# MartinPippel/DAmar

Hardware: AMD Instinct MI355X
Metric: aligned base-pairs/sec (daligner block-vs-block) (higher is better)
Workload: dtype int32

## Files before the change

### damar_amd/csrc/kernels/kernels.h

```cpp
#ifndef DAMAR_KERNELS_H
#define DAMAR_KERNELS_H

#include "dev_common.h"

size_t damar_scan_workspace_bytes(u64 n);
void   damar_exclusive_scan_u32(const u32 *in, u32 *out, u64 n, void *work, u64 *total_dev, hipStream_t st);
#define DAMAR_SCAN_TILE 4096
void   damar_tile_offsets_u32(const u32 *in, u64 n, void *work, u64 *total_dev, hipStream_t st);
void   damar_scan_tile_counts(u32 *tcount, u32 ntiles, u64 *total_dev, hipStream_t st);
size_t damar_sort_workspace_bytes(u64 n);
void   damar_sort_set_threads(int threads);
const u32 *damar_sort_error_word(const void *work);
int    damar_radix_sort_keys_u64(u64 *k0, u64 *k1, u64 n, int lobit, int hibit, void *work, hipStream_t st);
void   damar_radix_sort_split_u64(u64 *k0, u64 *k1, u64 n, int lobit, int hibit, u32 *ohi, u32 *olo, void *work,
                                  hipStream_t st);
int    damar_radix_sort_u32(u32 *k0, u32 *v0, u32 *k1, u32 *v1, u64 n, int nbits, void *work, hipStream_t st);
int    damar_radix_sort_keys_u32(u32 *k0, u32 *k1, u64 n, int nbits, void *work, hipStream_t st);
int    damar_radix_sort_u64(u64 *k0, u32 *v0, u64 *k1, u32 *v1, u64 n, int nbits, void *work, hipStream_t st);

enum { DAMAR_PILE_COVER = 0, DAMAR_PILE_REPEAT = 1, DAMAR_PILE_TANDEM = 2 };
#define DAMAR_PILE_ERR_RANGE 1u
typedef struct
{
  const long long *pile_off;
// ... 110 lines not shown

void damar_preload_index(void);  void damar_preload_scan(void);  void damar_preload_sort(void);
void damar_preload_merge(void);  void damar_preload_report(void);
void damar_sort_set_prio(int on);
void damar_merge_set_prio(int on);
void damar_index_set_prio(int on);
void damar_launch_kmer_tuples(const DevBlock *blk, int kmer, u32 nkmers, void *codes, int wide, u32 *pos, hipStream_t st);
void damar_launch_mask_flags(const DevBlock *blk, int kmer, const u32 *pos, u32 n, u32 *keep, hipStream_t st);
void damar_launch_biased_tuples(const DevBlock *blk, int kmer, const int *logbase, void *codes, int wide, u32 *pos,
                                u32 *keep, hipStream_t st);
void damar_launch_suppress_flags(const void *codes, int wide, u32 n, int suppress, u32 *keep, hipStream_t st);
void damar_launch_compact_pairs(const void *k, int wide, const u32 *v, const u32 *keep, const u32 *off, u32 n,
                                void *ko, u32 *vo, hipStream_t st);

void damar_launch_tandem_links(const DevBlock *blk, int kmer, const void *codes, int wide, const u32 *pos, u32 n,
                               int *dist, hipStream_t st);

typedef struct
{ const void *acode;  const u32 *apos;  u32 alen;
  const void *bcode;  const u32 *bpos;  u32 blen;
  int  wide;
  int  kbits;
  int  self, comp, identity;
  u32  limit;
  DevBlock ablk, bblk;
  int  pbits, abits;
  int  dbits;
  u32  b_lo, b_hi;
} MergeArgs;

typedef struct { u32 b0, b1, ja, ia;
                 u32 sh, pad[3]; } MergeTile;

size_t damar_merge_workspace_bytes(u32 alen);
u32   *damar_merge_tile_counts(void *work, u32 alen);
u32    damar_merge_tiles(u32 alen);
void   damar_launch_merge_count(const MergeArgs *m, void *work, unsigned long long *gram, u32 ngram, hipStream_t st);
void damar_launch_merge_emit(const MergeArgs *m, void *work, u64 nhits, u64 *keys, u32 *vals, u32 *pid, hipStream_t st);
void damar_launch_merge_bread_hist(const MergeArgs *m, void *work, unsigned long long *hist, hipStream_t st);
void damar_launch_merge_range(const MergeArgs *m, void *work, hipStream_t st);
void damar_launch_pair_heads_ids(const u32 *pids, u64 nhits, u64 off, u64 gtotal, int abits, int minhit, int nshift,
                                 u64 *send, u64 *bits, void *scan_work, u64 *total_dev, u32 *heads, hipStream_t st);
void damar_launch_pair_bitmap(const u32 *pids, const u32 *heads, u32 nheads, int abits, u32 b_lo, u32 b_hi, u32 *bitmap,
                              hipStream_t st);
void damar_launch_seed_cut_count(const u64 *keys, u64 nhits, int pbits, const u32 *bitmap, u32 *tcount, u64 *total_dev,
                                 hipStream_t st);
void damar_launch_seed_cut_scatter(const u64 *keys, const u32 *vals, u64 nhits, int pbits, const u32 *bitmap,
                                   const u32 *toff, u64 *okeys, u32 *ovals, hipStream_t st);
void damar_launch_pair_heads(const u64 *keys, u64 nhits, u64 off, u64 gtotal, int pbits, int abits, int minhit, int nshift,
                             u64 *send , u64 *bits, void *scan_work, u64 *total_dev,
                             u32 *heads, hipStream_t st);
void damar_launch_pair_work(u64 *keys, const u32 *vals, u64 nhits, u64 off, u64 gtotal, int ppos, int dbits, int abits, int minhit, int nshift,
                            u64 *send , u64 *bits, void *scan_work, u64 *total_dev ,
                            int binshift, int kmer, int hitmin, u32 b_lo, u32 b_hi, int unsorted, hipStream_t st);
size_t damar_order_runs_scratch_bytes(u64 nhits);
void damar_launch_order_runs(u64 *keys, u64 nhits, int ppos, int dbits, const u32 *work, u32 nwork, void *scratch, hipStream_t st);
void damar_launch_pair_work_expand(const u64 *bits, const void *scan_work, u64 nhits, u32 *work, hipStream_t st);
#define WORK_COST_BITS 16
#define WORK_COST_MAX  ((1u << WORK_COST_BITS) - 1)
void damar_launch_work_cost(const u64 *keys, const u32 *vals, u64 nhits, int pbits, int abits, int dbits, const u32 *aboff,
                            const u32 *bboff, const u32 *work, u32 nwork, u32 coarse, u32 *key, u32 *val, hipStream_t st);
void damar_launch_pair_screen(const u64 *keys, const u32 *vals, u64 nhits, int pbits, int dbits, const u32 *heads, u32 nheads,
                              int minhit, int binshift, int kmer, int hitmin, int abits, u32 b_lo, u32 b_hi, u32 *keep, hipStream_t st);
void damar_launch_compact_u32(const u32 *src, const u32 *keep, const u32 *off, u32 n, u32 *out, hipStream_t st);
void damar_launch_compact_index(const u32 *flags, const u32 *off, u64 n, u32 *out, hipStream_t st);

#ifdef __HIPCC__
__device__ __forceinline__ int seed_diag(u64 k, const u32 *__restrict__ vals, u64 i, u64 pmask, int dbits)
{ if (dbits)
    return (int) ((k >> dbits) & pmask) - (int) (k & ((1ull << dbits) - 1));
  return (int) vals[i];
}
#endif

typedef struct
{ int abpos, bbpos, aepos, bepos, diffs;
  int atlen, btlen;
  int aread, bread;
  u32 item, seq;
  u32 toff;
} LaRecord;

typedef struct
{
  const u64 *keys;  const u32 *vals;  u64 nhits;
  const u32 *work;  u32 nwork;
  DevBlock ablk, bblk;
  int  pbits, abits, dbits;
  int  kmer, hitmin, binshift, minhit;
// ... 134 lines not shown
```

### damar_amd/csrc/kernels/seed_merge.hip

```cpp
#include "dev_common.h"
#include "kernels.h"

SEED_PRIO_VAR(g_merge_prio, 0)
SEED_PRIO_SETTER(damar_merge_set_prio, g_merge_prio)


__device__ __forceinline__ u32 count_below(const u32 *__restrict__ bpos, u32 jb, u32 ib, u32 bound)
{ u32 a = jb, b = ib;
  while (a < b)
    { u32 m = (a + b) >> 1;
      if (bpos[m] < bound) a = m + 1; else b = m;
    }
  return a - jb;
}


#ifndef MT_PER
#define MT_PER  4
#endif
#define MT_A    (MT_PER * 256)
#define MT_BCAP (3 * MT_A)
#define MT_HITS 4
#define MT_NBK  2048

template <typename CodeT>
__device__ __forceinline__ u32 lower_bound_c(const CodeT *c, u32 lo, u32 hi, CodeT x)
{ while (lo < hi)
    { const u32 mid = (lo + hi) >> 1;
      if (c[mid] < x) lo = mid + 1; else hi = mid;
    }
  return lo;
}
template <typename CodeT>
__device__ __forceinline__ u32 upper_bound_c(const CodeT *c, u32 lo, u32 hi, CodeT x)
{ while (lo < hi)
    { const u32 mid = (lo + hi) >> 1;
      if (c[mid] <= x) lo = mid + 1; else hi = mid;
    }
  return lo;
}

#define MT_SMP 8192
template <typename CodeT>
__global__ __launch_bounds__(256)
void merge_tiles(MergeArgs m, u32 ntiles, MergeTile *__restrict__ tiles)
{ SEED_PRIO(g_merge_prio);
  constexpr u32 NS = sizeof(CodeT) == 4 ? MT_SMP : MT_SMP / 2;
  __shared__ CodeT smp[NS];
  const CodeT *acode = (const CodeT *) m.acode, *bcode = (const CodeT *) m.bcode;
  const u32 stride = (m.blen + NS - 1) / NS;
  if (m.blen > 0)
    for (u32 j = threadIdx.x; j < NS; j += 256)
      { const u64 e = (u64) (j + 1) * stride - 1;
        smp[j] = bcode[e < m.blen ? (u32) e : m.blen - 1];
      }
  __syncthreads();
  const u32 t = blockIdx.x * 256u + threadIdx.x;
  if (t >= ntiles)
    return;
  const u32 a0 = t * (u32) MT_A, a1 = min(m.alen, a0 + (u32) MT_A);
  const CodeT c0 = acode[a0], c1 = acode[a1 - 1];
  MergeTile tl;
  tl.b0 = tl.b1 = m.blen;
  if (m.blen > 0)
    { u32 lo = 0, hi = NS;
      while (lo < hi)
        { const u32 mid = (lo + hi) >> 1;
          if (smp[mid] < c0) lo = mid + 1; else hi = mid;
        }
      u32 l0 = m.blen, h0 = m.blen, l1 = m.blen, h1 = m.blen;
      if (lo < NS)
        { const u64 s0 = (u64) lo * stride;
          l0 = (u32) s0;  h0 = (u32) min((u64) m.blen, s0 + stride);
        }
      lo = 0;  hi = NS;
      while (lo < hi)
        { const u32 mid = (lo + hi) >> 1;
          if (smp[mid] <= c1) lo = mid + 1; else hi = mid;
        }
      if (lo < NS)
        { const u64 s0 = (u64) lo * stride;
          l1 = (u32) s0;  h1 = (u32) min((u64) m.blen, s0 + stride);
        }
// ... 318 lines not shown
    }
  if (threadIdx.x == 0)
    tcount[tile] = (T64 > 0xffffffffull) ? 0xffffffffu : (u32) T64;
  typedef u32 V4 __attribute__((ext_vector_type(4)));
  if (nv == MT_PER && MT_PER == 4)
    { V4 vc, vj;
#pragma unroll
      for (int k = 0; k < 4; k++)
        { vc[k] = n[k];  vj[k] = tl.b0 + jb[k]; }
      *(V4 *) (cnt + a0 + e0) = vc;
      *(V4 *) (jbg + a0 + e0) = vj;
    }
  else
    {
#pragma unroll
      for (int k = 0; k < MT_PER; k++)
        if (k < nv)
          { cnt[a0 + e0 + k] = n[k];
            jbg[a0 + e0 + k] = tl.b0 + jb[k];
          }
    }
}

static_assert(MT_BCAP + 16 < (1 << 16), "a packed entry holds the piece-relative start and the hits in 16 bits each");
struct MergeFastArgs
{ const void *acode, *bcode;
  const u32  *apos, *bpos;
  u32 alen, blen;
  int self, identity, comp, rpbits;
};

template <typename CodeT>
__global__ __launch_bounds__(256, 8)
void merge_fast(MergeFastArgs m, MergeTile *__restrict__ tiles, u32 *__restrict__ tcount, u32 *__restrict__ cnt)
{ SEED_PRIO(g_merge_prio);
  __shared__ __attribute__((aligned(16))) CodeT sb[MT_BCAP + 16 / sizeof(CodeT)];
  __shared__ __attribute__((aligned(16))) u16 first[MT_NBK];
  __shared__ u32 wsum[4];
  __shared__ u32 deep;
  const CodeT *acode = (const CodeT *) m.acode, *bcode = (const CodeT *) m.bcode;
  const u32 tile = blockIdx.x;
  const MergeTile tl = tiles[tile];
  const u32 a0 = tile * (u32) MT_A, a1 = min(m.alen, a0 + (u32) MT_A), nat = a1 - a0;
  const u32 nbt = tl.b1 - tl.b0;
  if (nbt > MT_BCAP || (m.self && m.rpbits == 0))
    { if (threadIdx.x == 0)
        tiles[tile].pad[0] = 1;
      return;
    }
  const u32 e0 = threadIdx.x * MT_PER;
  const int nv = (e0 >= nat) ? 0 : (int) min((u32) MT_PER, nat - e0);
  const u32 sh = tl.sh, nmax = tl.pad[1];
  constexpr u32 VPK = 16 / sizeof(CodeT);
  typedef CodeT VecT __attribute__((ext_vector_type(16 / sizeof(CodeT))));
  typedef u32 V4 __attribute__((ext_vector_type(4)));

  const CodeT c0 = acode[a0];
  CodeT a[MT_PER];
  if (nv == MT_PER)
    {
#pragma unroll
      for (int q = 0; q < MT_PER / (int) VPK; q++)
        { const VecT v = ((const VecT *) (acode + a0 + e0))[q];
#pragma unroll
          for (int e = 0; e < (int) VPK; e++)
            a[q * VPK + e] = v[e];
        }
    }
  else
    {
#pragma unroll
      for (int k = 0; k < MT_PER; k++)
        a[k] = (k < nv) ? acode[a0 + e0 + k] : (CodeT) 0;
    }
  const u32 b0a = tl.b0 & ~(VPK - 1), shf = tl.b0 - b0a;
  { const u32 nvec = (tl.b1 - b0a + VPK - 1) / VPK;
    const u32 whole = (m.blen - b0a) / VPK;
    VecT v[MT_BCAP / (int) VPK / 256 + 1];
#pragma unroll
    for (int r = 0; r < MT_BCAP / (int) VPK / 256 + 1; r++)
// ... 52 lines not shown
                  while (q < nbt && B[q] == c)
                    { q += 1;
                      if (++steps == 4) { q = upper_bound_c<CodeT>(B, q, nbt, c);  break; }
                    }
                  jb[k] = p;  n[k] = q - p;
                }
            }
          longest = max(longest, n[k]);
        }
    }
  if (longest > nmax)
    deep = 1;
  u32 sum = 0;
  if (m.self)
    { const int rp = m.rpbits;
#pragma unroll
      for (int k = 0; k < MT_PER; k++)
        if (n[k] > 0)
          { const u32 p = m.apos[a0 + e0 + k], ra = p >> rp;
            u32 bound = m.identity ? (m.comp ? (ra + 1) << rp : p) : ra << rp;
            if (!(m.identity && m.comp && ((ra + 1) >> (32 - rp)) != 0))
              n[k] = count_below(m.bpos, tl.b0 + jb[k], tl.b0 + jb[k] + n[k], bound);
          }
    }
#pragma unroll
  for (int k = 0; k < MT_PER; k++)
    sum += n[k];
  sum = (u32) wave_sum_i((int) sum);
  if (lane_id() == 0)
    wsum[threadIdx.x >> 6] = sum;
  __syncthreads();
  if (deep)
    { if (threadIdx.x == 0)
        tiles[tile].pad[0] = 1;
      return;
    }
  if (threadIdx.x == 0)
    { tcount[tile] = wsum[0] + wsum[1] + wsum[2] + wsum[3];
      tiles[tile].pad[2] = 1;
    }
  if (nv == MT_PER && MT_PER == 4)
    { V4 vc;
#pragma unroll
      for (int k = 0; k < 4; k++)
        vc[k] = (n[k] << 16) | jb[k];
      *(V4 *) (cnt + a0 + e0) = vc;
    }
  else
    {
#pragma unroll
      for (int k = 0; k < MT_PER; k++)
        if (k < nv)
          cnt[a0 + e0 + k] = (n[k] << 16) | jb[k];
    }
}

template <typename CodeT>
__global__ __launch_bounds__(256, 8)
void merge_sweep(MergeArgs m, const MergeTile *__restrict__ tiles, u32 *__restrict__ tcount, u32 *__restrict__ cnt,
                 u32 *__restrict__ jbg, unsigned long long *__restrict__ gram, u32 ngram, int only_flagged)
{ SEED_PRIO(g_merge_prio);
  __shared__ __attribute__((aligned(16))) CodeT sb[MT_BCAP + 16 / sizeof(CodeT)];
  __shared__ u32 loc[MT_A + 1];
  __shared__ u32 sjb[2];
  __shared__ u32 sw4[4];
  __shared__ u64 red[4];
  const MergeTile tl = tiles[blockIdx.x];
  if (only_flagged && tl.pad[0] == 0)
    return;
  if (tl.b1 - tl.b0 <= MT_BCAP)
    merge_sweep_tile<CodeT, true>(m, tl, blockIdx.x, tcount, cnt, jbg, gram, ngram, sb, loc, sjb, sw4, red);
  else
    merge_sweep_tile<CodeT, false>(m, tl, blockIdx.x, tcount, cnt, jbg, gram, ngram, sb, loc, sjb, sw4, red);
}

__global__ __launch_bounds__(256, 8)
void merge_emit(MergeArgs m, const MergeTile *__restrict__ tiles, const u32 *__restrict__ cnt, const u32 *__restrict__ jbg,
                const u32 *__restrict__ toff, u64 nhits, u64 *__restrict__ keys, u32 *__restrict__ vals, u32 *__restrict__ pid)
{ SEED_PRIO(g_merge_prio);
  __shared__ u32 loc[MT_A + 1];
  __shared__ u32 sjb[MT_A];
  __shared__ u32 sw4[4];
  const int l = lane_id(), w = threadIdx.x >> 6;
  const u32 tile = blockIdx.x;
  const u32 a0 = tile * (u32) MT_A, a1 = min(m.alen, a0 + (u32) MT_A), nat = a1 - a0;
  const u32 e0 = threadIdx.x * MT_PER;
  const u64 h0 = toff[tile];
  const u64 hn = (tile + 1 < gridDim.x) ? (u64) toff[tile + 1] : nhits;
  if (hn == h0)
    return;
  u32 n[MT_PER], s = 0;
  const bool packed = tiles[tile].pad[2] != 0;
  const u32 pb0 = tiles[tile].b0;
#pragma unroll
  for (int k = 0; k < MT_PER; k++)
    { const bool ok = e0 + k < nat;
      const u32 w = ok ? cnt[a0 + e0 + k] : 0;
      n[k] = packed ? w >> 16 : w;
      sjb[e0 + k] = !ok ? 0 : packed ? pb0 + (w & 0xffffu) : jbg[a0 + e0 + k];
      s += n[k];
    }
  u32 inc = (u32) wave_incl_scan_i((int) s);
  if (l == 63) sw4[w] = inc;
  __syncthreads();
  u32 ex = inc - s;
  for (int i = 0; i < 4; i++)
// ... 147 lines not shown
{ SEED_PRIO(g_merge_prio);
  __shared__ u64 red[4];
  const u32 tile = blockIdx.x;
  const u32 a0 = tile * (u32) MT_A, a1 = min(m.alen, a0 + (u32) MT_A);
  const bool packed = tiles[tile].pad[2] != 0;
  const u32 pb0 = tiles[tile].b0;
  u64 sum = 0;
  for (u32 i = a0 + threadIdx.x; i < a1; i += 256)
    { const u32 v = cnt[i];
      const u32 n = packed ? v >> 16 : v;
      if (n == 0)
        continue;
      const u32 jb = packed ? pb0 + (v & 0xffffu) : jbg[i];
      const u32 lo = count_reads_below(m, jb, n, m.b_lo), hi = count_reads_below(m, jb, n, m.b_hi);
      const u32 nn = hi > lo ? hi - lo : 0;
      if (packed)
        cnt[i] = (nn << 16) | (jb + lo - pb0);
      else
        { cnt[i] = nn;
          jbg[i] = jb + lo;
        }
      sum += nn;
    }
  const u64 T64 = block_sum_u64(sum, red);
  if (threadIdx.x == 0)
    tcount[tile] = (T64 > 0xffffffffull) ? 0xffffffffu : (u32) T64;
}


static size_t mw_tiles(u32 alen)  { return ((size_t) alen + MT_A - 1) / MT_A; }
static size_t mw_off_counts(u32 alen) { return (mw_tiles(alen) * sizeof(MergeTile) + 255) & ~(size_t) 255; }
static size_t mw_off_cnt(u32 alen)    { return mw_off_counts(alen) + (((mw_tiles(alen) + 1) * sizeof(u32) + 255) & ~(size_t) 255); }
static size_t mw_off_jb(u32 alen)     { return mw_off_cnt(alen) + (((size_t) alen * sizeof(u32) + 255) & ~(size_t) 255); }

size_t damar_merge_workspace_bytes(u32 alen)
{ return mw_off_jb(alen) + (((size_t) alen * sizeof(u32) + 255) & ~(size_t) 255); }

u32 *damar_merge_tile_counts(void *work, u32 alen) { return (u32 *) ((char *) work + mw_off_counts(alen)); }

u32 damar_merge_tiles(u32 alen) { return (u32) mw_tiles(alen); }

void damar_launch_merge_count(const MergeArgs *m, void *work, unsigned long long *gram, u32 ngram, hipStream_t st)
{ if (m->alen == 0)
    return;
  const u32 ntiles = (u32) mw_tiles(m->alen);
  MergeTile *tiles = (MergeTile *) work;
  u32 *tcount = damar_merge_tile_counts(work, m->alen);
  u32 *cnt = (u32 *) ((char *) work + mw_off_cnt(m->alen)), *jb = (u32 *) ((char *) work + mw_off_jb(m->alen));
  static int general = -1;
  if (general < 0)
    general = getenv("DAMAR_MERGE_GENERAL") != NULL;
  const bool fast = gram == NULL && !general;
  MergeFastArgs f;
  f.acode = m->acode;  f.bcode = m->bcode;  f.apos = m->apos;  f.bpos = m->bpos;  f.alen = m->alen;  f.blen = m->blen;
  f.self = m->self;  f.identity = m->identity;  f.comp = m->comp;  f.rpbits = m->ablk.rpbits;
  if (m->wide)
    { hipLaunchKernelGGL(merge_tiles<u64>, dim3((ntiles + 255) / 256), dim3(256), 0, st, *m, ntiles, tiles);
      if (fast)
        hipLaunchKernelGGL(merge_fast<u64>, dim3(ntiles), dim3(256), 0, st, f, tiles, tcount, cnt);
      hipLaunchKernelGGL(merge_sweep<u64>, dim3(ntiles), dim3(256), 0, st, *m, tiles, tcount, cnt, jb, gram, ngram, fast ? 1 : 0);
    }
  else
    { hipLaunchKernelGGL(merge_tiles<u32>, dim3((ntiles + 255) / 256), dim3(256), 0, st, *m, ntiles, tiles);
      if (fast)
        hipLaunchKernelGGL(merge_fast<u32>, dim3(ntiles), dim3(256), 0, st, f, tiles, tcount, cnt);
      hipLaunchKernelGGL(merge_sweep<u32>, dim3(ntiles), dim3(256), 0, st, *m, tiles, tcount, cnt, jb, gram, ngram, fast ? 1 : 0);
    }
}

void damar_launch_merge_emit(const MergeArgs *m, void *work, u64 nhits, u64 *keys, u32 *vals, u32 *pid, hipStream_t st)
{ if (nhits == 0)
    return;
  const u32 ntiles = (u32) mw_tiles(m->alen);
  const u32 *toff = damar_merge_tile_counts(work, m->alen);
  const u32 *cnt = (const u32 *) ((char *) work + mw_off_cnt(m->alen)), *jb = (const u32 *) ((char *) work + mw_off_jb(m->alen));
  hipLaunchKernelGGL(merge_emit, dim3(ntiles), dim3(256), 0, st, *m, (const MergeTile *) work, cnt, jb, toff, nhits, keys, vals, pid);
}

void damar_launch_merge_bread_hist(const MergeArgs *m, void *work, unsigned long long *hist, hipStream_t st)
{ if (m->alen == 0)
    return;
  const u32 ntiles = (u32) mw_tiles(m->alen);
  const u32 *cnt = (const u32 *) ((char *) work + mw_off_cnt(m->alen)), *jb = (const u32 *) ((char *) work + mw_off_jb(m->alen));
  hipLaunchKernelGGL(merge_bread_hist, dim3(ntiles), dim3(256), 0, st, *m, (const MergeTile *) work, cnt, jb, hist);
}

void damar_launch_merge_range(const MergeArgs *m, void *work, hipStream_t st)
{ if (m->alen == 0)
    return;
  const u32 ntiles = (u32) mw_tiles(m->alen);
  u32 *tcount = damar_merge_tile_counts(work, m->alen);
  u32 *cnt = (u32 *) ((char *) work + mw_off_cnt(m->alen)), *jb = (u32 *) ((char *) work + mw_off_jb(m->alen));
  hipLaunchKernelGGL(merge_range, dim3(ntiles), dim3(256), 0, st, *m, (const MergeTile *) work, tcount, cnt, jb);
}

#define SCREEN_MAX   48
#define SCREEN_PANEL 50000
template <typename K>
__global__ __launch_bounds__(64)
// ... 572 lines not shown
{ u32 n = 0;
  for (;;)
    { const u64 x = i + (u64) n + (u64) l;
      const u64 same = __ballot(x < nhits && (keys[x] >> pshift) == pr);
      if (same != ~0ull)
        return n + (u32) __ffsll((long long) ~same) - 1u;
      n += 64;
      if (n > maxrun)
        return n;
    }
}

__global__ __launch_bounds__(256)
void order_probe(const u64 *__restrict__ keys, u64 nhits, int ppos, int dbits, const u64 *__restrict__ bits, u64 *__restrict__ flag,
                 u32 maxrun)
{ SEED_PRIO(g_merge_prio);
  __shared__ u16 hl[DAMAR_SCAN_TILE];
  __shared__ u32 nh;
  const int  l = lane_id();
  const u64  base = (u64) blockIdx.x * DAMAR_SCAN_TILE;
  if (threadIdx.x == 0)
    nh = 0;
  __syncthreads();
  if (threadIdx.x < DAMAR_SCAN_TILE / 64)
    { u64 w = bits[(base >> 6) + threadIdx.x];
      while (w)
        { const int b = __ffsll((long long) w) - 1;
          w &= w - 1;
          hl[atomicAdd(&nh, 1u)] = (u16) (threadIdx.x * 64u + (u32) b);
        }
    }
  __syncthreads();
  const u32 n_h = nh;
  bool over = false;
  for (u32 h = threadIdx.x >> 6; h < n_h; h += 4)
    { const u64 i = base + hl[h];
      over |= run_length(keys, nhits, i, ppos + dbits, maxrun, l, keys[i] >> (ppos + dbits)) > maxrun;
    }
  if (over && l == 0)
    atomicOr((unsigned long long *) flag, 1ull);
}

template <u32 J>
__device__ __forceinline__ u32 lane_xor(u32 v)
{ if constexpr (J == 1)
    return (u32) __builtin_amdgcn_update_dpp(0, (int) v, 0xB1, 0xf, 0xf, true);
  else if constexpr (J == 2)
    return (u32) __builtin_amdgcn_update_dpp(0, (int) v, 0x4E, 0xf, 0xf, true);
  else if constexpr (J == 8)
    return (u32) __builtin_amdgcn_update_dpp(0, (int) v, 0x128, 0xf, 0xf, true);
  else if constexpr (J == 4 || J == 16)
    return (u32) __builtin_amdgcn_ds_swizzle((int) v, (int) (0x1f | (J << 10)));
  else
    return (u32) __shfl_xor((int) v, (int) J);
}

template <int K, u32 K2, u32 JJ>
__device__ __forceinline__ void or_step(u32 (&c)[K], int l)
{ if constexpr (JJ >= 64)
    {
#pragma unroll
      for (int q = 0; q < K; q++)
        if ((q & (int) (JJ >> 6)) == 0)
          { const int  p  = q | (int) (JJ >> 6);
            const bool up = (((u32) q << 6) & K2) == 0;
            const u32  lo = min(c[q], c[p]), hi = max(c[q], c[p]);
            c[q] = up ? lo : hi;
            c[p] = up ? hi : lo;
          }
    }
  else
    {
#pragma unroll
// ... 126 lines not shown
          { for (u32 t = threadIdx.x; t < (P >> 1); t += 256)
              { const u32 ix = ((t & ~(jj - 1)) << 1) | (t & (jj - 1)), px = ix | jj;
                const bool up = (ix & k2) == 0;
                const u32 a = ck[ix], c = ck[px];
                if ((a > c) == up)
                  { ck[ix] = c;  ck[px] = a; }
              }
            __syncthreads();
          }
      for (u32 j = threadIdx.x; j < n; j += 256)
        keys[i + j] = rk[ck[j] & 2047u];
      __syncthreads();
    }
}

size_t damar_order_runs_scratch_bytes(u64 nhits)
{ return sizeof(u32) * (size_t) (2 * (nhits / (OR_WAVE + 1)) + 2); }

#ifdef OR_STATS
static void or_stats_print(void)
{ unsigned long long h[16];
  if (hipMemcpyFromSymbol(h, HIP_SYMBOL(g_or_hist), sizeof(h)) != hipSuccess)
    return;
  unsigned long long runs = 0;
  for (int b = 0; b <= 12; b++)
    runs += h[b];
  fprintf(stderr, "order_runs: %llu kept runs, %llu seeds in them\n", runs, h[13]);
  for (int b = 0; b <= 12; b++)
    if (h[b])
      fprintf(stderr, "  runs of %5d..%-5d %9llu  (%.3f %%)\n", b == 0 ? 1 : (1 << b) + 1, b == 12 ? 1 << 30 : 2 << b, h[b], 100. * h[b] / runs);
}
#endif

void damar_launch_order_runs(u64 *keys, u64 nhits, int ppos, int dbits, const u32 *work, u32 nwork, void *scratch, hipStream_t st)
{ if (nwork == 0)
    return;
#ifdef OR_STATS
  static int reg = 0;
  if (!reg)
    { reg = 1;  atexit(or_stats_print); }
#endif
  u32 *lcount = (u32 *) scratch;
  HIP_CHECK(hipMemsetAsync(lcount, 0, sizeof(u32), st));
  const u32 slice = std::min<u32>(OR_SLICE, 4u * std::max<u32>(1u, nwork / 2048u));
  hipLaunchKernelGGL(order_waves, dim3((nwork + slice - 1) / slice), dim3(256), 0, st, keys, nhits, ppos, dbits, work, nwork, slice,
                     lcount, lcount + 2);
  if (nhits > OR_WAVE)
    { const u64 most = nhits / (OR_WAVE + 1);
      hipLaunchKernelGGL(order_long, dim3((u32) std::min<u64>(std::min<u64>(nwork, most), 1024)), dim3(256), 0, st, keys, ppos, dbits,
                         (const u32 *) lcount, (const u32 *) (lcount + 2));
    }
}

void damar_launch_pair_work(u64 *keys, const u32 *vals, u64 nhits, u64 off, u64 gtotal, int ppos, int dbits, int abits, int minhit, int nshift,
                            u64 *send, u64 *bits, void *scan_work, u64 *total_dev, int binshift, int kmer, int hitmin,
                            u32 b_lo, u32 b_hi, int unsorted, hipStream_t st)
{ HIP_CHECK(hipMemsetAsync(total_dev, 0, 2 * sizeof(u64), st));
  if (nhits == 0)
    return;
  if (nshift > 6)
    nshift = 6;
  const u32 ntiles = (u32) ((nhits + DAMAR_SCAN_TILE - 1) / DAMAR_SCAN_TILE);
  u32 *tcount = (u32 *) scan_work;
  if (nshift >= 0)
    hipLaunchKernelGGL(slice_ends<u64>, dim3(1), dim3(64), 0, st, keys, nhits, off, gtotal, abits + ppos + dbits, nshift, send);
  if (!unsorted)
    hipLaunchKernelGGL(pair_work_mark<false>, dim3(ntiles), dim3(256), 0, st, (const u64 *) keys, vals, nhits, ppos, dbits, abits, minhit,
                       nshift, (const u64 *) send, binshift, kmer, hitmin, b_lo, b_hi, bits, tcount);
  else
    { hipLaunchKernelGGL(pair_work_mark<true>, dim3(ntiles), dim3(256), 0, st, (const u64 *) keys, vals, nhits, ppos, dbits, abits, minhit,
                         nshift, (const u64 *) send, binshift, kmer, hitmin, b_lo, b_hi, bits, tcount);
      static int maxrun = -1;
      if (maxrun < 0)
        { const char *e = getenv("DAMAR_TEST_RUN_MAX");
          maxrun = (e && atoi(e) >= 2 && atoi(e) <= OR_MAX) ? atoi(e) : OR_MAX;
        }
      hipLaunchKernelGGL(order_probe, dim3(ntiles), dim3(256), 0, st, (const u64 *) keys, nhits, ppos, dbits, (const u64 *) bits, total_dev + 1,
                         (u32) maxrun);
    }
  damar_scan_tile_counts(tcount, ntiles, total_dev, st);
// ... 89 lines not shown
```

### damar_amd/csrc/kernels/sort_scan.hip

```cpp
#include "dev_common.h"
#include "kernels.h"

#define SCAN_THREADS 256
#define SCAN_ITEMS   16
#define SCAN_TILE    (SCAN_THREADS * SCAN_ITEMS)


__device__ __forceinline__ u32 block_excl_scan_256(u32 v, u32 *lds4, u32 *total)
{ int l = lane_id(), w = threadIdx.x >> 6;
  u32 inc = (u32) wave_incl_scan_i((int) v);
  if (l == 63) lds4[w] = inc;
  __syncthreads();
  u32 base = 0, tot = 0;
  for (int i = 0; i < 4; i++)
    { u32 s = lds4[i];
      if (i < w) base += s;
      tot += s;
    }
  __syncthreads();
  *total = tot;
  return base + inc - v;
}

__global__ __launch_bounds__(SCAN_THREADS)
void scan_tile_sums(const u32 *__restrict__ in, u64 n, u32 *__restrict__ tsum)
{ __shared__ u32 lds4[4];
  u64 base = (u64) blockIdx.x * SCAN_TILE + (u64) threadIdx.x * SCAN_ITEMS;
  u32 s = 0;
  for (int i = 0; i < SCAN_ITEMS; i++)
    if (base + i < n) s += in[base + i];
  u32 tot;
  block_excl_scan_256(s, lds4, &tot);
  if (threadIdx.x == 0) tsum[blockIdx.x] = tot;
}

__global__ __launch_bounds__(SCAN_THREADS)
void scan_tile_offsets(u32 *__restrict__ tsum, u32 ntiles, u64 *__restrict__ total)
{ __shared__ u32 lds4[4];
  u64 carry = 0;
  for (u32 b = 0; b < ntiles; b += SCAN_THREADS)
    { u32 i = b + threadIdx.x;
      u32 v = (i < ntiles) ? tsum[i] : 0, tot;
      u32 ex = block_excl_scan_256(v, lds4, &tot);
      if (i < ntiles) tsum[i] = (u32) (carry + ex);
      carry += tot;
    }
  if (threadIdx.x == 0) *total = carry;
}

__global__ __launch_bounds__(SCAN_THREADS)
void scan_tile_apply(const u32 *__restrict__ in, u32 *__restrict__ out, u64 n, const u32 *__restrict__ toff)
{ __shared__ u32 lds4[4];
  u64 base = (u64) blockIdx.x * SCAN_TILE + (u64) threadIdx.x * SCAN_ITEMS;
  u32 v[SCAN_ITEMS], s = 0;
  for (int i = 0; i < SCAN_ITEMS; i++)
    { v[i] = (base + i < n) ? in[base + i] : 0;
      s += v[i];
    }
  u32 tot;
  u32 ex = block_excl_scan_256(s, lds4, &tot) + toff[blockIdx.x];
  for (int i = 0; i < SCAN_ITEMS; i++)
    { if (base + i < n) out[base + i] = ex;
      ex += v[i];
    }
}

size_t damar_scan_workspace_bytes(u64 n)
{ u64 ntiles = (n + SCAN_TILE - 1) / SCAN_TILE;
  return ((((size_t) (ntiles + 1) * sizeof(u32)) + 63) & ~(size_t) 63) + 64;
}

void damar_exclusive_scan_u32(const u32 *in, u32 *out, u64 n, void *work, u64 *total_dev, hipStream_t st)
{ u32 ntiles = (u32) ((n + SCAN_TILE - 1) / SCAN_TILE);
  u32 *tsum = (u32 *) work;
  if (n == 0)
    { HIP_CHECK(hipMemsetAsync(total_dev, 0, sizeof(u64), st));
      return;
// ... 26 lines not shown
```

### damar_amd/csrc/shim.hip

```cpp
#include <algorithm>
#include <vector>
#include <deque>
#include <string>
#include <thread>
#include <atomic>
#include <mutex>
#include <condition_variable>
#include <functional>
#include <string.h>
#include <unistd.h>

#include "kernels/dev_common.h"
#include <ctype.h>
#include "kernels/kernels.h"

extern "C" {
#include "damar_filter.h"
#include "damar_hip.h"
#include "host/damar_host.h"
}

#define MAXGRAM 10000

static void die(void)
// ... 2120 lines not shown
      flags = (u32 *) arena_take(&G_tmp2, sizeof(u32) * (size_t) nsurv);
      foff  = (u32 *) arena_take(&G_tmp2, std::max(sizeof(u32) * (size_t) nsurv, bit_words_bytes(nsurv)));
      scw2  = arena_take(&G_tmp2, damar_scan_workspace_bytes(nsurv));
      sends = (u64 *) arena_take(&G_tmp2, 64 * sizeof(u64));
      damar_launch_seed_cut_scatter(uk, m.dbits ? NULL : uv, total, m.pbits + m.dbits, bitmap, (const u32 *) scc, k0, v0, G_st);
      int side = m.dbits ? damar_radix_sort_keys_u64(k0, k1, nsurv, m.dbits, m.dbits + sbits, sw2, G_st)
                         : damar_radix_sort_u64(k0, v0, k1, v1, nsurv, sbits, sw2, G_st);
      sort_check(sw2);
      keys = side ? k1 : k0;
      vals = side ? v1 : v0;
      if (keys != pk)
        { fprintf(stderr, "damar: internal error, the seed sort ended on the wrong side\n");
          die();
        }
      total  = nsurv;
      hshift = -1;
    }
  stage("seed_sort");
  tick(2);

  u64 nwork64 = 0;
  u32 *work = NULL;
  if (!two_step)
    {
      u64 got[2] = { 0, 0 };
      if (cut)
        psort = false;
      damar_launch_pair_work(keys, vals, total, s_off, s_all, m.pbits, m.dbits, m.abits, minhit, hshift, sends, (u64 *) foff ,
                             scw2, tot, P_binshift, P_kmer, P_hitmin, P_bread_lo, P_bread_hi, psort ? 1 : 0, G_st);
      stage("run_heads");
      tick(3);
      HIP_CHECK(hipMemcpyAsync(got, tot, 2 * sizeof(u64), hipMemcpyDeviceToHost, G_st));
      stream_wait(G_st);
      if (psort && got[1] != 0)
        {
          G_cnt[7] += 1;
          u64 *other = (keys == tk) ? NULL : tk;
          if (other == NULL || resort_ws == NULL)
            { fprintf(stderr, "damar: internal error, no room to sort the seeds again\n");
              die();
            }
          int side = damar_radix_sort_keys_u64(keys, other, total, m.dbits, m.dbits + sbits, resort_ws, G_st);
          sort_check(resort_ws);
          if (side)
            HIP_CHECK(hipMemcpyAsync(keys, other, sizeof(u64) * (size_t) total, hipMemcpyDeviceToDevice, G_st));
          damar_launch_pair_work(keys, vals, total, s_off, s_all, m.pbits, m.dbits, m.abits, minhit, hshift, sends, (u64 *) foff, scw2, tot,
                                 P_binshift, P_kmer, P_hitmin, P_bread_lo, P_bread_hi, 0, G_st);
          HIP_CHECK(hipMemcpyAsync(got, tot, 2 * sizeof(u64), hipMemcpyDeviceToHost, G_st));
          stream_wait(G_st);
          psort = false;
        }
      nwork64 = got[0];
      arena_reserve(&G_ord, 5 * pad256(sizeof(u32) * (size_t) nwork64) + pad256(damar_sort_workspace_bytes(nwork64)) + 8192);
      work = (u32 *) arena_take(&G_ord, sizeof(u32) * ((size_t) nwork64 + 1));
      if (nwork64 > 0)
        { damar_launch_pair_work_expand((const u64 *) foff, scw2, total, work, G_st);
          if (psort)
            damar_launch_order_runs(keys, total, m.pbits, m.dbits, work, (u32) nwork64, order_ws, G_st);
        }
      stage("work_list");
    }
  else
    { u32 *heads = (u32 *) tk;
      damar_launch_pair_heads(keys, total, s_off, s_all, m.pbits + m.dbits, m.abits, minhit, hshift, sends, (u64 *) foff ,
                              scw2, tot, heads, G_st);
      stage("run_heads");
      HIP_CHECK(hipMemcpyAsync(&nwork64, tot, sizeof(u64), hipMemcpyDeviceToHost, G_st));
      HIP_CHECK(hipStreamSynchronize(G_st));
      const u32 nheads = (u32) nwork64;
      arena_reserve(&G_ord, 5 * pad256(sizeof(u32) * (size_t) nheads) + pad256(damar_sort_workspace_bytes(nheads)) + 8192);
      work = (u32 *) arena_take(&G_ord, sizeof(u32) * ((size_t) nheads + 1));
      nwork64 = 0;
      if (nheads > 0)
        { damar_launch_pair_screen(keys, vals, total, m.pbits, m.dbits, heads, nheads, minhit, P_binshift, P_kmer, P_hitmin, m.abits,
                                   P_bread_lo, P_bread_hi, flags, G_st);
          damar_exclusive_scan_u32(flags, foff, nheads, scw2, tot, G_st);
          damar_launch_compact_u32(heads, flags, foff, nheads, work, G_st);
          stage("work_list");
          HIP_CHECK(hipMemcpyAsync(&nwork64, tot, sizeof(u64), hipMemcpyDeviceToHost, G_st));
        }
    }
  if (two_step)
    { tick(3);
      HIP_CHECK(hipStreamSynchronize(G_st));
    }
  sort_verify();
  const u32 nwork = (u32) nwork64;
  G_ms[DAMAR_T_MERGE] += lap(0, 1);
  G_ms[DAMAR_T_SSORT] += lap(1, 2);
  G_ms[DAMAR_T_WORK]  += lap(2, 3);
  G_cnt[0] += nhits;  G_cnt[1] += nwork;
// ... 823 lines not shown
  damar_dev_block *b = damar_block_upload(ablock);
  damar_match_self(ablock, b, settings, NULL);
  damar_block_free(b);
}


extern "C" int damar_last_slabs(int *b_lo, int64 *hits, int cap)
{ const int n = G_plan.n;
  for (int i = 0; i < n && i < cap; i++)
    { if (b_lo) b_lo[i] = G_plan.b_lo[(size_t) i];
      if (hits) hits[i] = G_plan.hits[(size_t) i];
    }
  if (b_lo != NULL && n <= cap && (size_t) n < G_plan.b_lo.size())
    b_lo[n] = G_plan.b_lo[(size_t) n];
  return n;
}

extern "C" void damar_slab_totals(int64 *out)
{ out[0] = G_slab_tot[0];  out[1] = G_slab_tot[1]; }

extern "C" int damar_order_runs_test(uint64 *keys, int64 nhits, int ppos, int dbits, const uint32 *work, int nwork)
{ finish_all();
  ensure_init();
  if (nhits <= 0 || nwork <= 0)
    return 0;
  u64  *dk;
  u32  *dw;
  void *sc;
  HIP_CHECK(hipMalloc((void **) &dk, sizeof(u64) * (size_t) nhits));
  HIP_CHECK(hipMalloc((void **) &dw, sizeof(u32) * (size_t) nwork));
  HIP_CHECK(hipMalloc(&sc, damar_order_runs_scratch_bytes((u64) nhits)));
  HIP_CHECK(hipMemcpy(dk, keys, sizeof(u64) * (size_t) nhits, hipMemcpyHostToDevice));
  HIP_CHECK(hipMemcpy(dw, work, sizeof(u32) * (size_t) nwork, hipMemcpyHostToDevice));
  damar_launch_order_runs(dk, (u64) nhits, ppos, dbits, dw, (u32) nwork, sc, G_st);
  HIP_CHECK(hipStreamSynchronize(G_st));
  HIP_CHECK(hipMemcpy(keys, dk, sizeof(u64) * (size_t) nhits, hipMemcpyDeviceToHost));
  HIP_CHECK(hipFree(dk));  HIP_CHECK(hipFree(dw));  HIP_CHECK(hipFree(sc));
  return 0;
}

extern "C" int64 damar_last_seeds(void *out, int64 cap)
{ struct SP { int diag, apos, aread, bread; } *sp = (SP *) out;
  if (out == NULL)
    { G_keep_seeds = (cap != 0);
      return 0;
    }
  int64 n = (int64) G_seed_keys.size();
  for (int64 i = 0; i < n && i < cap; i++)
    { u64 k = G_seed_keys[(size_t) i];
      const int bpos = (int) (k & ((1ull << G_seed_dbits) - 1));
      k >>= G_seed_dbits;
      sp[i].apos  = (int) (k & ((1ull << G_seed_pbits) - 1));
      sp[i].aread = (int) ((k >> G_seed_pbits) & ((1ull << G_seed_abits) - 1));
      sp[i].bread = (int) (k >> (G_seed_pbits + G_seed_abits));
      sp[i].diag  = G_seed_dbits ? sp[i].apos - bpos : (int) G_seed_vals[(size_t) i];
    }
  return n;
}

extern "C" int damar_local_alignment_batch_opts(damar_dev_block *ablk, damar_dev_block *bblk, int comp,
                                                Align_Spec *spec, const int *tasks, int ntasks,
                                                int *paths, int64 *trace_off, uint16 *traces, int64 trace_cap,
                                                int t8, int *t8_fell_back, int *wide_tasks)
{ finish_all();
  ensure_init();
  if (t8_fell_back) *t8_fell_back = 0;
  if (wide_tasks)   *wide_tasks = 0;
// ... 935 lines not shown
```

Baseline: 53.87 billion.

## Sweep only fallback merge tiles via worklist and skip idle long-run ordering

merge_fast now appends each tile it cannot handle to a device worklist. A grid-strided merge_sweep_list kernel then processes only those tiles, replacing the full-grid merge_sweep launch in which most blocks exit early. The run-length check now sets a separate 'long run' flag bit, so order_long is launched only when some run is longer than a wave. The tile-offset scan is also rewritten to handle several items per thread with u64 accumulation. Both skips can be turned off with an environment variable, and correctness depends on the atomic list and flag bits being set reliably.

```diff
diff --git a/damar_amd/csrc/kernels/kernels.h b/damar_amd/csrc/kernels/kernels.h
--- a/damar_amd/csrc/kernels/kernels.h
+++ b/damar_amd/csrc/kernels/kernels.h
@@ -166,6 +166,7 @@
 typedef struct { u32 b0, b1, ja, ia;
                  u32 sh, pad[3]; } MergeTile;
 
+int    damar_seed_idle_skip(void);
 size_t damar_merge_workspace_bytes(u32 alen);
 u32   *damar_merge_tile_counts(void *work, u32 alen);
 u32    damar_merge_tiles(u32 alen);
@@ -184,11 +185,14 @@
 void damar_launch_pair_heads(const u64 *keys, u64 nhits, u64 off, u64 gtotal, int pbits, int abits, int minhit, int nshift,
                              u64 *send , u64 *bits, void *scan_work, u64 *total_dev,
                              u32 *heads, hipStream_t st);
+#define DAMAR_RUN_OVER 1u
+#define DAMAR_RUN_LONG 2u
 void damar_launch_pair_work(u64 *keys, const u32 *vals, u64 nhits, u64 off, u64 gtotal, int ppos, int dbits, int abits, int minhit, int nshift,
                             u64 *send , u64 *bits, void *scan_work, u64 *total_dev ,
                             int binshift, int kmer, int hitmin, u32 b_lo, u32 b_hi, int unsorted, hipStream_t st);
 size_t damar_order_runs_scratch_bytes(u64 nhits);
-void damar_launch_order_runs(u64 *keys, u64 nhits, int ppos, int dbits, const u32 *work, u32 nwork, void *scratch, hipStream_t st);
+void damar_launch_order_runs(u64 *keys, u64 nhits, int ppos, int dbits, const u32 *work, u32 nwork, void *scratch, int maybe_long,
+                             hipStream_t st);
 void damar_launch_pair_work_expand(const u64 *bits, const void *scan_work, u64 nhits, u32 *work, hipStream_t st);
 #define WORK_COST_BITS 16
 #define WORK_COST_MAX  ((1u << WORK_COST_BITS) - 1)
diff --git a/damar_amd/csrc/kernels/seed_merge.hip b/damar_amd/csrc/kernels/seed_merge.hip
--- a/damar_amd/csrc/kernels/seed_merge.hip
+++ b/damar_amd/csrc/kernels/seed_merge.hip
@@ -3,6 +3,15 @@
 
 SEED_PRIO_VAR(g_merge_prio, 0)
 SEED_PRIO_SETTER(damar_merge_set_prio, g_merge_prio)
+
+int damar_seed_idle_skip(void)
+{ static int on = -1;
+  if (on < 0)
+    { const char *e = getenv("DAMAR_SEED_SKIP");
+      on = (e == NULL || atoi(e) != 0) ? 1 : 0;
+    }
+  return on;
+}
 
 
 __device__ __forceinline__ u32 count_below(const u32 *__restrict__ bpos, u32 jb, u32 ib, u32 bound)
@@ -43,12 +52,14 @@
 #define MT_SMP 8192
 template <typename CodeT>
 __global__ __launch_bounds__(256)
-void merge_tiles(MergeArgs m, u32 ntiles, MergeTile *__restrict__ tiles)
+void merge_tiles(MergeArgs m, u32 ntiles, MergeTile *__restrict__ tiles, u32 *__restrict__ fcount)
 { SEED_PRIO(g_merge_prio);
   constexpr u32 NS = sizeof(CodeT) == 4 ? MT_SMP : MT_SMP / 2;
   __shared__ CodeT smp[NS];
   const CodeT *acode = (const CodeT *) m.acode, *bcode = (const CodeT *) m.bcode;
   const u32 stride = (m.blen + NS - 1) / NS;
+  if (blockIdx.x == 0 && threadIdx.x == 0)
+    *fcount = 0;
   if (m.blen > 0)
     for (u32 j = threadIdx.x; j < NS; j += 256)
       { const u64 e = (u64) (j + 1) * stride - 1;
@@ -433,7 +444,8 @@
 
 template <typename CodeT>
 __global__ __launch_bounds__(256, 8)
-void merge_fast(MergeFastArgs m, MergeTile *__restrict__ tiles, u32 *__restrict__ tcount, u32 *__restrict__ cnt)
+void merge_fast(MergeFastArgs m, MergeTile *__restrict__ tiles, u32 *__restrict__ tcount, u32 *__restrict__ cnt,
+                u32 *__restrict__ fcount, u32 *__restrict__ flist)
 { SEED_PRIO(g_merge_prio);
   __shared__ __attribute__((aligned(16))) CodeT sb[MT_BCAP + 16 / sizeof(CodeT)];
   __shared__ __attribute__((aligned(16))) u16 first[MT_NBK];
@@ -446,7 +458,9 @@
   const u32 nbt = tl.b1 - tl.b0;
   if (nbt > MT_BCAP || (m.self && m.rpbits == 0))
     { if (threadIdx.x == 0)
-        tiles[tile].pad[0] = 1;
+        { tiles[tile].pad[0] = 1;
+          flist[atomicAdd(fcount, 1u)] = tile;
+        }
       return;
     }
   const u32 e0 = threadIdx.x * MT_PER;
@@ -565,7 +579,9 @@
   __syncthreads();
   if (deep)
     { if (threadIdx.x == 0)
-        tiles[tile].pad[0] = 1;
+        { tiles[tile].pad[0] = 1;
+          flist[atomicAdd(fcount, 1u)] = tile;
+        }
       return;
     }
   if (threadIdx.x == 0)
@@ -605,6 +621,29 @@
     merge_sweep_tile<CodeT, true>(m, tl, blockIdx.x, tcount, cnt, jbg, gram, ngram, sb, loc, sjb, sw4, red);
   else
     merge_sweep_tile<CodeT, false>(m, tl, blockIdx.x, tcount, cnt, jbg, gram, ngram, sb, loc, sjb, sw4, red);
+}
+
+#define MT_LIST_GRID 512
+template <typename CodeT>
+__global__ __launch_bounds__(256)
+void merge_sweep_list(MergeArgs m, const MergeTile *__restrict__ tiles, u32 *__restrict__ tcount, u32 *__restrict__ cnt,
+                      u32 *__restrict__ jbg, const u32 *__restrict__ fcount, const u32 *__restrict__ flist)
+{ SEED_PRIO(g_merge_prio);
+  __shared__ __attribute__((aligned(16))) CodeT sb[MT_BCAP + 16 / sizeof(CodeT)];
+  __shared__ u32 loc[MT_A + 1];
+  __shared__ u32 sjb[2];
+  __shared__ u32 sw4[4];
+  __shared__ u64 red[4];
+  const u32 nf = *fcount;
+  for (u32 f = blockIdx.x; f < nf; f += gridDim.x)
+    { const u32 tile = flist[f];
+      const MergeTile tl = tiles[tile];
+      if (tl.b1 - tl.b0 <= MT_BCAP)
+        merge_sweep_tile<CodeT, true>(m, tl, tile, tcount, cnt, jbg, NULL, 0, sb, loc, sjb, sw4, red);
+      else
+        merge_sweep_tile<CodeT, false>(m, tl, tile, tcount, cnt, jbg, NULL, 0, sb, loc, sjb, sw4, red);
+      __syncthreads();
+    }
 }
 
 __global__ __launch_bounds__(256, 8)
@@ -818,9 +857,10 @@
 static size_t mw_off_counts(u32 alen) { return (mw_tiles(alen) * sizeof(MergeTile) + 255) & ~(size_t) 255; }
 static size_t mw_off_cnt(u32 alen)    { return mw_off_counts(alen) + (((mw_tiles(alen) + 1) * sizeof(u32) + 255) & ~(size_t) 255); }
 static size_t mw_off_jb(u32 alen)     { return mw_off_cnt(alen) + (((size_t) alen * sizeof(u32) + 255) & ~(size_t) 255); }
+static size_t mw_off_flag(u32 alen)   { return mw_off_jb(alen) + (((size_t) alen * sizeof(u32) + 255) & ~(size_t) 255); }
 
 size_t damar_merge_workspace_bytes(u32 alen)
-{ return mw_off_jb(alen) + (((size_t) alen * sizeof(u32) + 255) & ~(size_t) 255); }
+{ return mw_off_flag(alen) + (((mw_tiles(alen) + 1) * sizeof(u32) + 255) & ~(size_t) 255); }
 
 u32 *damar_merge_tile_counts(void *work, u32 alen) { return (u32 *) ((char *) work + mw_off_counts(alen)); }
 
@@ -837,20 +877,31 @@
   if (general < 0)
     general = getenv("DAMAR_MERGE_GENERAL") != NULL;
   const bool fast = gram == NULL && !general;
+  const bool listed = fast && damar_seed_idle_skip();
+  u32 *fcount = (u32 *) ((char *) work + mw_off_flag(m->alen)), *flist = fcount + 1;
+  const u32 lgrid = std::min<u32>(ntiles, MT_LIST_GRID);
   MergeFastArgs f;
   f.acode = m->acode;  f.bcode = m->bcode;  f.apos = m->apos;  f.bpos = m->bpos;  f.alen = m->alen;  f.blen = m->blen;
   f.self = m->self;  f.identity = m->identity;  f.comp = m->comp;  f.rpbits = m->ablk.rpbits;
   if (m->wide)
-    { hipLaunchKernelGGL(merge_tiles<u64>, dim3((ntiles + 255) / 256), dim3(256), 0, st, *m, ntiles, tiles);
+    { hipLaunchKernelGGL(merge_tiles<u64>, dim3((ntiles + 255) / 256), dim3(256), 0, st, *m, ntiles, tiles, fcount);
       if (fast)
-        hipLaunchKernelGGL(merge_fast<u64>, dim3(ntiles), dim3(256), 0, st, f, tiles, tcount, cnt);
-      hipLaunchKernelGGL(merge_sweep<u64>, dim3(ntiles), dim3(256), 0, st, *m, tiles, tcount, cnt, jb, gram, ngram, fast ? 1 : 0);
+        hipLaunchKernelGGL(merge_fast<u64>, dim3(ntiles), dim3(256), 0, st, f, tiles, tcount, cnt, fcount, flist);
+      if (listed)
+        hipLaunchKernelGGL(merge_sweep_list<u64>, dim3(lgrid), dim3(256), 0, st, *m, tiles, tcount, cnt, jb, (const u32 *) fcount,
+                           (const u32 *) flist);
+      else
+        hipLaunchKernelGGL(merge_sweep<u64>, dim3(ntiles), dim3(256), 0, st, *m, tiles, tcount, cnt, jb, gram, ngram, fast ? 1 : 0);
     }
   else
-    { hipLaunchKernelGGL(merge_tiles<u32>, dim3((ntiles + 255) / 256), dim3(256), 0, st, *m, ntiles, tiles);
+    { hipLaunchKernelGGL(merge_tiles<u32>, dim3((ntiles + 255) / 256), dim3(256), 0, st, *m, ntiles, tiles, fcount);
       if (fast)
-        hipLaunchKernelGGL(merge_fast<u32>, dim3(ntiles), dim3(256), 0, st, f, tiles, tcount, cnt);
-      hipLaunchKernelGGL(merge_sweep<u32>, dim3(ntiles), dim3(256), 0, st, *m, tiles, tcount, cnt, jb, gram, ngram, fast ? 1 : 0);
+        hipLaunchKernelGGL(merge_fast<u32>, dim3(ntiles), dim3(256), 0, st, f, tiles, tcount, cnt, fcount, flist);
+      if (listed)
+        hipLaunchKernelGGL(merge_sweep_list<u32>, dim3(lgrid), dim3(256), 0, st, *m, tiles, tcount, cnt, jb, (const u32 *) fcount,
+                           (const u32 *) flist);
+      else
+        hipLaunchKernelGGL(merge_sweep<u32>, dim3(ntiles), dim3(256), 0, st, *m, tiles, tcount, cnt, jb, gram, ngram, fast ? 1 : 0);
     }
 }
 
@@ -1489,13 +1540,15 @@
     }
   __syncthreads();
   const u32 n_h = nh;
-  bool over = false;
+  bool over = false, lng = false;
   for (u32 h = threadIdx.x >> 6; h < n_h; h += 4)
     { const u64 i = base + hl[h];
-      over |= run_length(keys, nhits, i, ppos + dbits, maxrun, l, keys[i] >> (ppos + dbits)) > maxrun;
-    }
-  if (over && l == 0)
-    atomicOr((unsigned long long *) flag, 1ull);
+      const u32 n = run_length(keys, nhits, i, ppos + dbits, maxrun, l, keys[i] >> (ppos + dbits));
+      over |= n > maxrun;
+      lng  |= n > OR_WAVE || n > maxrun;
+    }
+  if ((over || lng) && l == 0)
+    atomicOr((unsigned long long *) flag, (unsigned long long) ((over ? DAMAR_RUN_OVER : 0u) | (lng ? DAMAR_RUN_LONG : 0u)));
 }
 
 template <u32 J>
@@ -1688,7 +1741,8 @@
 }
 #endif
 
-void damar_launch_order_runs(u64 *keys, u64 nhits, int ppos, int dbits, const u32 *work, u32 nwork, void *scratch, hipStream_t st)
+void damar_launch_order_runs(u64 *keys, u64 nhits, int ppos, int dbits, const u32 *work, u32 nwork, void *scratch, int maybe_long,
+                             hipStream_t st)
 { if (nwork == 0)
     return;
 #ifdef OR_STATS
@@ -1701,7 +1755,7 @@
   const u32 slice = std::min<u32>(OR_SLICE, 4u * std::max<u32>(1u, nwork / 2048u));
   hipLaunchKernelGGL(order_waves, dim3((nwork + slice - 1) / slice), dim3(256), 0, st, keys, nhits, ppos, dbits, work, nwork, slice,
                      lcount, lcount + 2);
-  if (nhits > OR_WAVE)
+  if (nhits > OR_WAVE && (maybe_long || !damar_seed_idle_skip()))
     { const u64 most = nhits / (OR_WAVE + 1);
       hipLaunchKernelGGL(order_long, dim3((u32) std::min<u64>(std::min<u64>(nwork, most), 1024)), dim3(256), 0, st, keys, ppos, dbits,
                          (const u32 *) lcount, (const u32 *) (lcount + 2));
diff --git a/damar_amd/csrc/kernels/sort_scan.hip b/damar_amd/csrc/kernels/sort_scan.hip
--- a/damar_amd/csrc/kernels/sort_scan.hip
+++ b/damar_amd/csrc/kernels/sort_scan.hip
@@ -36,13 +36,37 @@
 
 __global__ __launch_bounds__(SCAN_THREADS)
 void scan_tile_offsets(u32 *__restrict__ tsum, u32 ntiles, u64 *__restrict__ total)
-{ __shared__ u32 lds4[4];
+{ __shared__ u64 lds4[4];
+  const int l = lane_id(), w = threadIdx.x >> 6;
   u64 carry = 0;
-  for (u32 b = 0; b < ntiles; b += SCAN_THREADS)
-    { u32 i = b + threadIdx.x;
-      u32 v = (i < ntiles) ? tsum[i] : 0, tot;
-      u32 ex = block_excl_scan_256(v, lds4, &tot);
-      if (i < ntiles) tsum[i] = (u32) (carry + ex);
+  for (u64 b = 0; b < ntiles; b += SCAN_TILE)
+    { const u64 i0 = b + (u64) threadIdx.x * SCAN_ITEMS;
+      u32 v[SCAN_ITEMS];
+      u64 s = 0, tot = 0;
+#pragma unroll
+      for (int i = 0; i < SCAN_ITEMS; i++)
+        v[i] = (i0 + i < ntiles) ? tsum[i0 + i] : 0;
+#pragma unroll
+      for (int i = 0; i < SCAN_ITEMS; i++)
+        s += v[i];
+      u64 inc = s;
+      for (int o = 1; o < 64; o <<= 1)
+        { const u64 t = (u64) __shfl_up((long long) inc, o);
+          if (l >= o) inc += t;
+        }
+      if (l == 63) lds4[w] = inc;
+      __syncthreads();
+      u64 ex = carry + inc - s;
+      for (int i = 0; i < 4; i++)
+        { if (i < w) ex += lds4[i];
+          tot += lds4[i];
+        }
+      __syncthreads();
+#pragma unroll
+      for (int i = 0; i < SCAN_ITEMS; i++)
+        { if (i0 + i < ntiles) tsum[i0 + i] = (u32) ex;
+          ex += v[i];
+        }
       carry += tot;
     }
   if (threadIdx.x == 0) *total = carry;
diff --git a/damar_amd/csrc/shim.hip b/damar_amd/csrc/shim.hip
--- a/damar_amd/csrc/shim.hip
+++ b/damar_amd/csrc/shim.hip
@@ -2176,7 +2176,7 @@
       tick(3);
       HIP_CHECK(hipMemcpyAsync(got, tot, 2 * sizeof(u64), hipMemcpyDeviceToHost, G_st));
       stream_wait(G_st);
-      if (psort && got[1] != 0)
+      if (psort && (got[1] & DAMAR_RUN_OVER) != 0)
         {
           G_cnt[7] += 1;
           u64 *other = (keys == tk) ? NULL : tk;
@@ -2200,7 +2200,8 @@
       if (nwork64 > 0)
         { damar_launch_pair_work_expand((const u64 *) foff, scw2, total, work, G_st);
           if (psort)
-            damar_launch_order_runs(keys, total, m.pbits, m.dbits, work, (u32) nwork64, order_ws, G_st);
+            damar_launch_order_runs(keys, total, m.pbits, m.dbits, work, (u32) nwork64, order_ws,
+                                    (got[1] & DAMAR_RUN_LONG) != 0, G_st);
         }
       stage("work_list");
     }
@@ -3090,7 +3091,7 @@
   HIP_CHECK(hipMalloc(&sc, damar_order_runs_scratch_bytes((u64) nhits)));
   HIP_CHECK(hipMemcpy(dk, keys, sizeof(u64) * (size_t) nhits, hipMemcpyHostToDevice));
   HIP_CHECK(hipMemcpy(dw, work, sizeof(u32) * (size_t) nwork, hipMemcpyHostToDevice));
-  damar_launch_order_runs(dk, (u64) nhits, ppos, dbits, dw, (u32) nwork, sc, G_st);
+  damar_launch_order_runs(dk, (u64) nhits, ppos, dbits, dw, (u32) nwork, sc, 1, G_st);
   HIP_CHECK(hipStreamSynchronize(G_st));
   HIP_CHECK(hipMemcpy(keys, dk, sizeof(u64) * (size_t) nhits, hipMemcpyDeviceToHost));
   HIP_CHECK(hipFree(dk));  HIP_CHECK(hipFree(dw));  HIP_CHECK(hipFree(sc));
```

New measurement: 53.85 billion. No clear change (-0.0%).
